# Ray0089/geometric-aware-dense-matching

Measured on AMD Instinct MI355X. Metric: rgbd_crops_per_sec_geomatch_fwd, higher is better.
Workload: dtype bf16x3/f32acc

## Files before the change

### geometric_aware_dense_matching_amd/_lib.py

```python
import ctypes
import os
import subprocess

_PKG = os.path.dirname(os.path.abspath(__file__))
LIB_PATH = os.path.join(_PKG, "libgdm_hip.so")
CSRC = os.path.join(_PKG, "csrc")

_vp = ctypes.c_void_p
_i = ctypes.c_int
_f = ctypes.c_float
_sz = ctypes.c_size_t

GDM_RANSAC_MAX_H = 4096


class KnnJob(ctypes.Structure):
    _fields_ = [("support", _vp), ("query", _vp), ("idx", _vp), ("d2", _vp),
                ("support_bstride", ctypes.c_int64), ("query_bstride", ctypes.c_int64),
                ("S", ctypes.c_int32), ("Q", ctypes.c_int32), ("K", ctypes.c_int32), ("grid_w", ctypes.c_int32)]


class PwSeg(ctypes.Structure):
    _fields_ = [("x", _vp), ("idx", _vp), ("C", ctypes.c_int32), ("n_src", ctypes.c_int32)]

# ... 22 lines not shown
    "gdm_labelstat_idx_hip": (_i, [_i, _i, _i, _i, _i, _vp, _vp, _vp, _vp]),
    "gdm_group_gather_hip": (_i, [_vp, _vp, _i, _i, _i, _i, _i, _vp, _vp]),
    "gdm_group_gather_bwd2_hip": (_i, [_vp, ctypes.c_long, _vp, _i, _i, _i, _i, _i, _vp, _vp]),
    "gdm_gather_max_hip": (_i, [_vp, _vp, _i, _i, _i, _i, _i, _vp, _vp, _vp]),
    "gdm_gather_max_bwd_hip": (_i, [_vp, _vp, _i, _i, _i, _i, _vp, _vp]),
    "gdm_rel_pos_enc_hip": (_i, [_vp, _vp, _i, _i, _i, _vp, _vp]),
    "gdm_att_pool_hip": (_i, [_vp, _vp, _i, _i, _i, _i, _vp, _vp]),
    "gdm_att_pool_bwd_hip": (_i, [_vp, _vp, _vp, _i, _i, _i, _i, _vp, _vp, _vp]),
    "gdm_match_workspace_bytes": (_sz, [_i, _i, _i]),
    "gdm_match_hip": (_i, [_vp, _vp, _i, _i, _i, _i, _i, _vp, _vp, _vp, _vp, _sz, _vp]),
    "gdm_match_rows_bytes": (_sz, [_i]),
    "gdm_match_partial_bytes": (_sz, [_i, _i]),
    "gdm_match_pack_hip": (_i, [_vp, _i, _i, _i, _i, _vp, _vp]),
    "gdm_match_pack2_hip": (_i, [_vp, _i, _i, _vp, _vp, _i, _i, _vp, _i, _i, _vp]),
    "gdm_match_packed_hip": (_i, [_vp, _vp, _i, _i, _i, _vp, _vp, _vp, _vp, _sz, _vp]),
    "gdm_seg_mask_hip": (_i, [_vp, _i, _i, _vp, _vp, _vp]),
    "gdm_spline_aggregate_hip": (_i, [_vp, _vp, _vp, _vp, _vp, _vp, _i, _i, _i, _i, _vp, _vp]),
    "gdm_spline_aggregate_bwd_hip": (_i, [_vp, _vp, _vp, _vp, _i, _i, _i, _vp, _vp]),
    "gdm_spline_direct3_hip": (_i, [_vp, _vp, _vp, _vp, _vp, _vp, _vp, _i, _i, _i, _i, _i, _vp, _vp, _vp, _vp]),
    "gdm_gemm_grouped_hip": (_i, [_vp, _vp, _vp, _vp, _i, _i, _i, _i, _vp, _vp]),
    "gdm_spline_pairs_aggregate3_hip": (_i, [_vp, _vp, _vp, _vp, _vp, _vp, _i, _i, _i, _vp, _vp, _vp, _vp]),
    "gdm_upsample_bilinear_hip": (_i, [_vp, ctypes.c_long, _i, _i, _i, _i, _vp, _vp]),
    "gdm_upsample_bilinear_bwd_hip": (_i, [_vp, ctypes.c_long, _i, _i, _i, _i, _vp, _vp]),
    "gdm_topk_rows_hip": (_i, [_vp, ctypes.c_long, _i, _i, _vp, _vp, _vp]),
    "gdm_topk_negdist_hip": (_i, [_vp, _vp, _i, _i, _i, _vp, _vp]),
    "gdm_edge_feature_hip": (_i, [_vp, _vp, _i, _i, _i, _i, _vp, _vp]),
    "gdm_edge_feature_bwd_hip": (_i, [_vp, _vp, _i, _i, _i, _i, _vp, _vp]),
    "gdm_circle_rows_fwd_hip": (_i, [_vp, _i, _i, _vp, _vp, _vp, _vp, _f, _f, _f, _vp, _vp, _vp, _vp]),
    "gdm_circle_rows_bwd_hip": (_i, [_vp, _i, _i, _vp, _vp, _vp, _vp, _f, _f, _f, _vp, _vp, _vp, _vp, _vp]),
    "gdm_circle_match_rows_bytes": (_sz, [_i]),
    "gdm_circle_match_tp_bytes": (_sz, [_i]),
    "gdm_circle_match_pack_hip": (_i, [_vp, _i, _vp, _vp, _vp, _vp]),
    "gdm_circle_match_nbr_hip": (_i, [_vp, _i, _f, _vp, _vp]),
    "gdm_circle_match_visbits_hip": (_i, [_vp, _i, _i, _vp, _vp]),
    "gdm_circle_match_nbr_items_hip": (_i, [_vp, _i, _vp, _i, _vp, _vp]),
    "gdm_circle_match_fwd2_hip": (_i, [_vp, _vp, _vp, _vp, _vp, _i, _i, _vp, _vp, _vp, _vp, _i, _vp, _i, _f, _f, _vp, _vp, _vp, _vp]),
    "gdm_circle_match_bwd2_hip": (_i, [_vp, _vp, _vp, _vp, _vp, _i, _i, _vp, _vp, _vp, _vp, _i, _vp, _i, _f, _f, _vp, _vp, _vp, _vp, _vp, _vp]),
    "gdm_circle_match_bwd_parts": (_i, [_i, _i]),
    "gdm_lfa_stage_hip": (_i, [_vp] * 13 + [_i, _i, _i, _i, _i, _f, _vp, _vp]),
    "gdm_kabsch_stats_hip": (_i, [_vp, ctypes.c_long, _i, _i, _vp, _vp, _vp, _i, _i, _i, _vp, _vp]),
    "gdm_kabsch_solve_hip": (_i, [_vp, _i, _i, _vp, _vp, _vp]),
    "gdm_ransac_workspace_bytes": (_sz, [_i, _i, _i]),
    "gdm_ransac_pose_hip": (_i, [_vp, ctypes.c_long, _i, _i, _vp, _vp, _vp, _vp, _i, _i, _i, _i, _f, ctypes.c_double, ctypes.c_uint32, _i,
                                 _vp, _sz, _vp, _vp, _vp, _vp, _vp]),
    "gdm_icp_transform_hip": (_i, [_vp, ctypes.c_long, _i, _i, _vp, _i, _i, _vp, _vp]),
    "gdm_icp_update_hip": (_i, [_vp, ctypes.c_long, _i, _i, _vp, _vp, _vp, _vp, _i, _i, _i, _f, ctypes.c_double, _i, _vp, _vp, _vp, _vp,
                                _vp]),
    "gdm_affine_act_maxk_hip": (_i, [_vp, _vp, _vp, ctypes.c_long, _i, ctypes.c_long, _i, _i, _f, _vp, _vp]),
    "gdm_prelu1_hip": (_i, [_vp, _vp, ctypes.c_long, _vp, _vp]),
    "gdm_prelu1_bwd_hip": (_i, [_vp, _vp, _vp, ctypes.c_long, _vp, _vp, _vp]),
    "gdm_affine_act_hip": (_i, [_vp, _vp, _vp, _vp, _vp, _vp, ctypes.c_long, _i, ctypes.c_long, _i, _f, _vp, _vp]),
    "gdm_upconv3x3_gather_hip": (_i, [_vp, _vp, _vp, _i, _i, _i, _i, _i, _i, _i, _f, _vp, _vp]),
    "gdm_upconv3x3_gather2_hip": (_i, [_vp, _vp, _vp, _i, _i, _i, _i, _i, _i, _i, _f, _vp, _vp, _vp]),
    "gdm_upconv3x3_gather_bwd_hip": (_i, [_vp, _i, _i, _i, _i, _i, _i, _vp, _vp]),
    "gdm_upconv_fused64_weight_bytes": (_sz, []),
    "gdm_upconv_fused64_pack_weight_hip": (_i, [_vp, _vp, _vp]),
    "gdm_upconv_fused64_hip": (_i, [_vp, _vp, _vp, _vp, _i, _i, _i, _i, _i, _i, _i, _f, _vp, _vp]),
    "gdm_psp_combine2_hip": (_i, [_vp, _vp, _i, _vp, _i, _vp, _i, _vp, _i, _vp, _i, _i, _i, _i, _vp, _vp, _vp]),
    "gdm_gather_add_affine_act2_hip": (_i, [_vp, _vp, _vp, _vp, _vp, _i, _i, _i, _i, _i, _f, _vp, _vp, _i, _vp]),
    "gdm_conv1x1_gather_add_act2_hip": (_i, [_vp, _vp, _vp, _vp, _vp, _vp, _i, _i, _i, ctypes.c_long, _i, _f, _i, _vp, _vp]),
    "gdm_conv64_gather_add_act_mfma2_hip": (_i, [_vp, _vp, _vp, _vp, _vp, _vp, _i, _i, ctypes.c_long, _i, _f, _i, _i, _vp, _vp, _i, _vp]),
    "gdm_conv3x3_act_bytes": (_sz, [_i, _i, _i, _i]),
    "gdm_conv3x3_weight_bytes": (_sz, [_i, _i]),
    "gdm_conv3x3_pack_weight_hip": (_i, [_vp, _i, _i, _vp, _vp]),
    "gdm_conv3x3_pack_act_hip": (_i, [_vp, _i, _i, _i, _i, _vp, _vp]),
    "gdm_conv3x3_packed_hip": (_i, [_vp, _vp, _vp, _vp, _vp, _i, _i, _i, _i, _i, _i, _vp, _vp]),
    "gdm_conv3x3_strided_hip": (_i, [_vp, _vp, _vp, _vp, _vp, _i, _i, _i, _i, _i, _i, _i, _vp, _vp, _vp]),
    "gdm_conv1x1_strided_hip": (_i, [_vp, _vp, _vp, _vp, _i, _i, _i, _i, _i, _i, _i, _vp, _vp]),
    "gdm_affine_relu_maxpool_hip": (_i, [_vp, _vp, _vp, _i, _i, _i, _i, _vp, _vp]),
    "gdm_conv1x1_logsoftmax_hip": (_i, [_vp, _vp, _vp, _i, _i, ctypes.c_long, _vp, _vp]),
    "gdm_pack_rows64_hip": (_i, [_vp, _i, _vp, _vp]),
    "gdm_upconv_final_points_hip": (_i, [_vp, _vp, _vp, _vp, _vp, _i, _f, _vp, _vp, _i, _i, _i, _i, _i, _i, _vp, _vp]),
    "gdm_psp_pools_hip": (_i, [_vp, ctypes.c_long, _i, _i, _vp, _vp, _vp, _vp, _vp]),
    "gdm_psp_pools_bwd_hip": (_i, [_vp, _vp, _vp, _vp, ctypes.c_long, _i, _i, _vp, _vp]),
    "gdm_conv1x1_weight_bytes": (_sz, [_i, _i]),
    "gdm_conv1x1_pack_weight_hip": (_i, [_vp, _i, _i, _vp, _vp]),
    "gdm_conv_pack_weight_dgrad_hip": (_i, [_vp, _i, _i, _i, _vp, _vp]),
    "gdm_conv1x1_packed_hip": (_i, [_vp, _vp, _vp, _vp, _i, _i, _i, _i, _i, _i, _i, _vp, _vp]),
    "gdm_depth_to_xyz_hip": (_i, [_vp, _vp, _vp, _i, _i, _i, _i, _vp, _vp]),
    "gdm_bn_sums_len": (ctypes.c_long, [_i, _i, ctypes.c_long]),
    "gdm_bn_stats_hip": (_i, [_vp, _i, _i, ctypes.c_long, _vp, _vp]),
    "gdm_bn_fwd_apply_hip": (_i, [_vp, _vp, _i, _vp, _vp, _i, _i, ctypes.c_long, _f, _f, _i, _f, _vp, _vp, _vp, _vp, _vp]),
    "gdm_bn_bwd_reduce_hip": (_i, [_vp, _vp, _vp, _i, _i, ctypes.c_long, _i, _f, _vp, _vp]),
    "gdm_bn_bwd_apply_hip": (_i, [_vp, _vp, _vp, _i, _vp, _vp, _i, _i, ctypes.c_long, _i, _f, _vp, _vp, _vp, _vp]),
    "gdm_point_heads2_hip": (_i, [_vp, _vp, _i, _vp, _vp, _i, _i, _i, _i, _vp, _vp, _vp, _vp, _i, _i, _vp, _vp, _i, _vp, _vp, _vp]),
    "gdm_pointwise2_hip": (_i, [ctypes.POINTER(PwSeg), _i, _vp, _i, _vp, _vp, _i, _i, _i, _i, _f, _vp, _i, _i, _i, _vp]),
    "gdm_pointwise_jobs_hip": (_i, [ctypes.POINTER(PwJob), _i, _i, _i, _i, _vp]),
    "gdm_pointwise_chain2_hip": (_i, [_vp, _vp, _vp, _vp, _i, _f, _vp, _vp, _vp, _i, _f, _i, _i, _i, _i, _i, _vp, _vp, _vp]),
    "gdm_stem_weight_bytes": (_sz, []),
    "gdm_stem_pack_weight_hip": (_i, [_vp, _vp, _vp]),
    "gdm_stem_hip": (_i, [_vp, _vp, _vp, _vp, _i, _i, _i, _vp, _vp, _vp]),
    "gdm_wgrad_x_bytes": (_sz, [_i, _i, _i, _i]),
    "gdm_wgrad_go_bytes": (_sz, [_i, _i, _i, _i]),
    "gdm_wgrad_pack_x_hip": (_i, [_vp, _i, _i, _i, _i, _vp, _vp]),
    "gdm_wgrad_pack_go_hip": (_i, [_vp, _i, _i, _i, _i, _vp, _vp]),
    "gdm_wgrad_x1_bytes": (_sz, [_i, _i, _i]),
    "gdm_wgrad_pack_x1_hip": (_i, [_vp, _i, _i, _i, _vp, _vp]),
    "gdm_mfma_probe_hip": (_i, [_i, _i, _i, _vp, _vp]),
    "gdm_mfma_probe_lds_hip": (_i, [_i, _i, _i, _vp, _vp]),
    "gdm_wgrad_direct_hip": (_i, [_vp, ctypes.c_long, _vp, ctypes.c_long, _i, _i, _i, _i, _i, _vp, _vp, _vp]),
    "gdm_conv1x1_packed_wb_hip": (_i, [_vp, _vp, ctypes.c_long, _i, _i, _i, _i, _i, _vp, _vp]),
    "gdm_copy_jobs_hip": (_i, [ctypes.POINTER(CopyJob), _i, _vp]),
}

_lib = None

# ... 80 lines not shown
```

### geometric_aware_dense_matching_amd/cnn.py

```python
import math
import os

import torch
import torch.nn as nn
import torch.nn.functional as F

from . import ops, settings
from .layers import act_code, cached_gemm_weight, folded_bn, fused_eval




def bn_act(bn, x, relu=None):
    if ops.bn_train_supported(x, bn):
        return ops.batch_norm_act_train(x, bn, ops.ACT_RELU if relu is not None else ops.ACT_NONE)
    y = bn(x)
    return relu(y) if relu is not None else y


def _conv3x3(cin, cout, stride=1, dilation=1):
    return nn.Conv2d(cin, cout, kernel_size=3, stride=stride, padding=dilation, dilation=dilation, bias=False)


class BasicBlock(nn.Module):
# ... 184 lines not shown
        sizes = [st[0].output_size[0] if isinstance(st[0].output_size, (tuple, list)) else st[0].output_size for st in self.stages]
        if (settings.USE_SPLIT_PSP_TRAIN and feats.is_cuda and feats.dtype == torch.float32 and sizes == [1, 2, 3, 6] and ops.psp_pools_supported(h, w)
                and (h * w) % 4 == 0 and feats.shape[0] * self.bottleneck.out_channels <= 65535 and h <= 64 and w <= 64):
            B, F_ = feats.shape[0], feats.shape[1]
            w2 = self.bottleneck.weight.view(self.bottleneck.out_channels, -1)
            g = ops.wx(w2[:, 4 * F_:], feats.reshape(B, F_, h * w)).view(B, -1, h, w)
            pools = ops.psp_pools(feats)
            ys = []
            for k, st in enumerate(self.stages):
                m = w2[:, k * F_:(k + 1) * F_] @ st[1].weight.view(F_, F_)
                ys.append(ops.wx(m, pools[k].reshape(B, F_, sizes[k] * sizes[k])).view(B, -1, sizes[k], sizes[k]))
            return ops.psp_combine_train(g, ys, self.bottleneck.bias)
        priors = [ops.upsample_bilinear(stage(feats), (h, w)) for stage in self.stages] + [feats]
        return self.relu(self.bottleneck(torch.cat(priors, 1)))


class Upsample2x(nn.Module):

    def forward(self, x):
        return ops.upsample_bilinear(x, (x.shape[2] * 2, x.shape[3] * 2))


class PSPUpsample(nn.Module):
    def __init__(self, cin, cout):
        super().__init__()
        self.conv = nn.Sequential(Upsample2x(), nn.Conv2d(cin, cout, 3, padding=1), nn.BatchNorm2d(cout), nn.PReLU())

    def _tap_major_weight(self):
        w = self.conv[1].weight
        key = (w._version, w.data_ptr())
        cache = self.__dict__.get("_gdm_wt")
        if cache is None or cache[0] != key:
            with torch.no_grad():
                wt = w.permute(2, 3, 0, 1).reshape(9 * w.shape[0], w.shape[1]).contiguous()
            cache = (key, wt)
            self.__dict__["_gdm_wt"] = cache
        return cache[1]

    def forward(self, x):
        if fused_eval(x, self):
            code = act_code(self.conv[3])
            conv = self.conv[1]
            if code is not None and x.shape[0] * conv.out_channels <= 65535 and conv.in_channels >= settings.UPCONV_MIN_CIN:
                Bx, Cin, Hx, Wx = x.shape
                if settings.USE_FUSED_UPCONV and Cin == 64 and conv.out_channels == 64 and Hx >= 2 and Wx >= 2 and Bx <= 65535:
                    w = conv.weight
                    key = (w._version, w.data_ptr())
                    cache = self.__dict__.get("_gdm_fused64")
                    if cache is None or cache[0] != key:
                        cache = (key, ops.upconv_fused64_pack_weight(w))
                        self.__dict__["_gdm_fused64"] = cache
                    scale, shift = folded_bn(self.conv[2], conv.bias)
                    return ops.upconv_fused64(x, cache[1], scale, shift, (Hx * 2, Wx * 2), code[0], code[1])
                if settings.USE_MFMA_GEMM and ops.gemm_supported(Cin, 9 * conv.out_channels, Hx * Wx):
                    wpk, c9 = cached_gemm_weight(self, "tap", self._tap_major_weight, (conv.weight,))
                    z = ops.gemm_bf16x3_map(x, wpk, c9)
                else:
                    z = ops.wx(self._tap_major_weight(), x.reshape(Bx, Cin, Hx * Wx)).view(Bx, -1, Hx, Wx)
                scale, shift = folded_bn(self.conv[2], conv.bias)
                return ops.upconv3x3_gather(z, scale, shift, conv.out_channels, (x.shape[2] * 2, x.shape[3] * 2), code[0], code[1],
                                            packed=settings.USE_MFMA_GEMM and settings.USE_PACKED_PRODUCERS and conv.out_channels % 128 == 0)
        act = self.conv[3]
        if x.is_cuda and isinstance(act, nn.PReLU) and act.weight.numel() == 1 and x.dtype == torch.float32:
            conv = self.conv[1]
            if settings.USE_LOWRES_UPCONV_TRAIN and ops.upconv_train_supported(x.shape[0], conv.out_channels) and conv.in_channels >= settings.UPCONV_MIN_CIN:
                Bx, Cin, Hx, Wx = x.shape
                w9 = conv.weight.permute(2, 3, 0, 1).reshape(9 * conv.out_channels, Cin)
                z = ops.wx(w9, x.reshape(Bx, Cin, Hx * Wx)).view(Bx, -1, Hx, Wx)
                y = bn_act(self.conv[2], ops.upconv3x3_gather_train(z, conv.bias, conv.out_channels, (Hx * 2, Wx * 2)))
            else:
                y = bn_act(self.conv[2], conv(self.conv[0](x)))
            if y.numel() % 4 == 0:
                return ops.prelu1(y, act.weight)
            return act(y)
        return self.conv(x)


class FinalStage(nn.Sequential):

    def forward(self, x):
        conv = self[0]
        if fused_eval(x, self) and conv.in_channels == 64 and conv.out_channels == 64 and x.shape[0] <= 65535:
            return ops.conv1x1_logsoftmax(x, conv.weight, conv.bias)
        if self.training and ops.conv1x1_train_supported(conv, x):
            return self[1](ops.conv1x1_train(conv, x))
        return nn.Sequential.forward(self, x)


class PSPNet(nn.Module):

    def __init__(self):
        super().__init__()
        self.feats = ResNet18Trunk()
        self.psp = PSPModule(512, 1024, (1, 2, 3, 6))
        self.drop_1 = nn.Dropout2d(p=0.3)
        self.up_1 = PSPUpsample(1024, 256)
        self.up_2 = PSPUpsample(256, 64)
        self.up_3 = PSPUpsample(64, 64)
        self.drop_2 = nn.Dropout2d(p=0.15)
        self.final = FinalStage(nn.Conv2d(64, 64, kernel_size=1), nn.LogSoftmax(dim=1))
```

### geometric_aware_dense_matching_amd/ops.py

```python
import ctypes
import os

import torch

from . import _lib, settings
from ._lib import KnnJob, check

MATCH_BF16X3 = 0
MATCH_F32 = 1


def _stream():
    return torch.cuda.current_stream().cuda_stream


_side_streams = {}


def side_stream(device, which=0):
    key = (device.index if device.index is not None else torch.cuda.current_device(), which)
    st = _side_streams.get(key)
    if st is None:
        st = torch.cuda.Stream(device=device)
        _side_streams[key] = st
# ... 687 lines not shown
    if not bn.affine or bn.momentum is None or not bn.track_running_stats:
        return False
    B, C = x.shape[0], x.shape[1]
    inner = x.numel() // max(B * C, 1)
    return B * C <= 65535 and inner >= 4 and inner % 4 == 0 and x.data_ptr() % 16 == 0 and B * inner > 1


def batch_norm_act_train(x, bn, act=ACT_NONE, slope=0.0):
    y = _BatchNormAct.apply(x, bn.weight, bn.bias, bn.running_mean, bn.running_var, bn.eps, bn.momentum, act, slope, _sync_group(bn))
    if bn.num_batches_tracked is not None:
        if _bn_counters is not None:
            _bn_counters.append(bn.num_batches_tracked)
        else:
            bn.num_batches_tracked.add_(1)
    return y


_bn_counters = None


class batched_bn_counters:

    def __enter__(self):
        global _bn_counters
        self.prev, _bn_counters = _bn_counters, []
        return self

    def __exit__(self, *exc):
        global _bn_counters
        pending, _bn_counters = _bn_counters, self.prev
        if pending:
            torch._foreach_add_(pending, 1)
        return False


def upconv3x3_gather(z, scale, shift, cout, out_size, act=ACT_NONE, slope=0.0, packed=False):
    z = _dev(z, torch.float32, "z")
    B, c9, H, W = z.shape
    assert c9 == 9 * cout
    OH, OW = int(out_size[0]), int(out_size[1])
    out = torch.empty((B, cout, OH, OW), dtype=torch.float32, device=z.device)
    if (packed and (cout == 64 or cout % 128 == 0) and OW % 32 == 0 and (B * OH * OW) % 256 == 0 and B * cout // 8 <= 65535
            and (OH, OW) == (2 * H, 2 * W)):
        opk = PackedAct(_packed_buffer(B, cout, OH, OW, z.device), (B, cout, OH, OW))
        check(_lib.lib().gdm_upconv3x3_gather2_hip(z.data_ptr(), scale.data_ptr(), shift.data_ptr(), B, cout, H, W, OH, OW, act,
                                                   float(slope), out.data_ptr(), opk.buf.data_ptr(), _stream()), "gdm_upconv3x3_gather2_hip")
        out._gdm_packed = opk
        return out
    check(_lib.lib().gdm_upconv3x3_gather_hip(z.data_ptr(), scale.data_ptr(), shift.data_ptr(), B, cout, H, W, OH, OW, act,
                                              float(slope), out.data_ptr(), _stream()), "gdm_upconv3x3_gather_hip")
    return out


def upconv_fused64_pack_weight(weight):
    w = _dev(weight.detach(), torch.float32, "weight")
    if tuple(w.shape) != (64, 64, 3, 3):
        raise ValueError("upconv_fused64_pack_weight: weight must be [64,64,3,3], got %s" % (tuple(w.shape),))
    L = _lib.lib()
    wpk = torch.empty(L.gdm_upconv_fused64_weight_bytes(), dtype=torch.uint8, device=w.device)
    check(L.gdm_upconv_fused64_pack_weight_hip(w.data_ptr(), wpk.data_ptr(), _stream()), "gdm_upconv_fused64_pack_weight_hip")
    return wpk


def upconv_fused64(x, wpk, scale, shift, out_size, act=0, slope=0.0):
    x = _dev(x, torch.float32, "x")
    B, C, H, W = x.shape
    OH, OW = int(out_size[0]), int(out_size[1])
    out = torch.empty((B, C, OH, OW), dtype=torch.float32, device=x.device)
    check(_lib.lib().gdm_upconv_fused64_hip(x.data_ptr(), wpk.data_ptr(), scale.data_ptr(), shift.data_ptr(), B, C, H, W, OH, OW, act,
                                            float(slope), out.data_ptr(), _stream()), "gdm_upconv_fused64_hip")
    return out


class _UpconvGather(torch.autograd.Function):

    @staticmethod
    def forward(ctx, z, bias, cout, OH, OW):
        z = z.contiguous()
        B, c9, H, W = z.shape
        ones = torch.ones(cout, dtype=torch.float32, device=z.device)
        shift = bias.detach().contiguous() if bias is not None else torch.zeros(cout, dtype=torch.float32, device=z.device)
        out = torch.empty((B, cout, OH, OW), dtype=torch.float32, device=z.device)
        check(_lib.lib().gdm_upconv3x3_gather_hip(z.data_ptr(), ones.data_ptr(), shift.data_ptr(), B, cout, H, W, OH, OW, ACT_NONE, 0.0,
                                                  out.data_ptr(), _stream()), "gdm_upconv3x3_gather_hip")
        ctx.shape = (B, cout, H, W, OH, OW)
        ctx.has_bias = bias is not None
        return out

    @staticmethod
    def backward(ctx, go):
        B, cout, H, W, OH, OW = ctx.shape
        go = go.contiguous()
        gz = torch.empty((B, 9 * cout, H, W), dtype=torch.float32, device=go.device)
        check(_lib.lib().gdm_upconv3x3_gather_bwd_hip(go.data_ptr(), B, cout, H, W, OH, OW, gz.data_ptr(), _stream()),
              "gdm_upconv3x3_gather_bwd_hip")
        return gz, (channel_sum(go) if ctx.has_bias else None), None, None, None


def upconv3x3_gather_train(z, bias, cout, out_size):
    z = _dev(z, torch.float32, "z")
    assert z.shape[1] == 9 * cout
    return _UpconvGather.apply(z, bias, cout, int(out_size[0]), int(out_size[1]))


def wx(w2d, x3):
    if torch.is_grad_enabled() and (w2d.requires_grad or x3.requires_grad) and x3.is_cuda and x3.dtype == torch.float32:
# ... 843 lines not shown
```

### geometric_aware_dense_matching_amd/settings.py

```python
import os


def _flag(name, default="1"):
    return os.environ.get(name, default) != "0"


USE_MFMA_CONV = _flag("GDM_MFMA_CONV")
USE_MFMA_CONV_TRAIN = _flag("GDM_MFMA_CONV_TRAIN")
USE_MFMA_GEMM = _flag("GDM_MFMA_GEMM")
USE_FUSED_UPCONV = _flag("GDM_FUSED_UPCONV")
USE_LOWRES_UPCONV_TRAIN = _flag("GDM_LOWRES_UPCONV_TRAIN")
USE_SPLIT_PSP_TRAIN = _flag("GDM_SPLIT_PSP_TRAIN")
USE_FUSED_LFA = _flag("GDM_FUSED_LFA")
USE_GROUPED_SPLINE = _flag("GDM_GROUPED_SPLINE")
USE_FUSED_BN_TRAIN = _flag("GDM_FUSED_BN_TRAIN")
USE_FUSED_SYNCBN = _flag("GDM_FUSED_SYNCBN")
USE_FUSED_MATCH_LOSS = _flag("GDM_FUSED_MATCH_LOSS")
USE_SIDE_STREAMS = _flag("GDM_SIDE_STREAMS", "0")
USE_SPARSE_FINAL = _flag("GDM_SPARSE_FINAL")
USE_FUSED_HEADS = _flag("GDM_FUSED_HEADS")
USE_MFMA_STRIDED = _flag("GDM_MFMA_STRIDED")
USE_POINTWISE = _flag("GDM_POINTWISE")
USE_OWN_STEM = _flag("GDM_OWN_STEM")
USE_GEMM_CONV1X1_TRAIN = _flag("GDM_GEMM_CONV1X1_TRAIN")
USE_MFMA_WGRAD = _flag("GDM_MFMA_WGRAD")
USE_MFMA_GEMM_TRAIN = _flag("GDM_MFMA_GEMM_TRAIN")
USE_GATHERED_FINAL = _flag("GDM_GATHERED_FINAL")
USE_DIRECT_WGRAD = _flag("GDM_DIRECT_WGRAD")
USE_FUSED_ADAM = _flag("GDM_FUSED_ADAM")
USE_POINTWISE_TRAIN = _flag("GDM_POINTWISE_TRAIN")
USE_POINT_CHAIN = _flag("GDM_POINT_CHAIN")
USE_PSP_JOBS = _flag("GDM_PSP_JOBS")
USE_PACKED_PRODUCERS = _flag("GDM_PACKED_PRODUCERS")
USE_TWO_STREAM_PIPELINE = _flag("GDM_TWO_STREAM_PIPELINE")
MESH_FORK_LATE = os.environ.get("GDM_MESH_FORK_LATE", "1") != "0"
PACK_MESH_ROWS = os.environ.get("GDM_PACK_MESH_ROWS", "1") != "0"
SIDE_PARTS = os.environ.get("GDM_SIDE_PARTS", "mesh,point,pyr").split(",")
STATIC_MATCH_ROWS = _flag("GDM_STATIC_MATCH_ROWS", "0")
UPCONV_MIN_CIN = int(os.environ.get("GDM_UPCONV_MIN_CIN", "0"))
SYNCBN_MIN_WORLD = 2

ALL_SWITCHES = ("USE_MFMA_CONV", "USE_MFMA_CONV_TRAIN", "USE_MFMA_GEMM", "USE_FUSED_UPCONV", "USE_LOWRES_UPCONV_TRAIN",
                "USE_SPLIT_PSP_TRAIN", "USE_FUSED_LFA", "USE_GROUPED_SPLINE", "USE_FUSED_BN_TRAIN", "USE_FUSED_SYNCBN",
                "USE_FUSED_MATCH_LOSS", "USE_SIDE_STREAMS", "USE_SPARSE_FINAL", "USE_FUSED_HEADS", "USE_MFMA_STRIDED", "USE_POINTWISE", "USE_OWN_STEM", "USE_GEMM_CONV1X1_TRAIN", "USE_MFMA_WGRAD", "USE_MFMA_GEMM_TRAIN", "USE_GATHERED_FINAL", "USE_DIRECT_WGRAD", "USE_PSP_JOBS", "USE_POINT_CHAIN", "USE_POINTWISE_TRAIN")
SPLIT_BF16_SWITCHES = ("USE_MFMA_CONV", "USE_MFMA_GEMM", "USE_FUSED_UPCONV", "USE_SPARSE_FINAL", "USE_FUSED_HEADS", "USE_MFMA_STRIDED",
                       "USE_OWN_STEM")
```

### include/gdm.h

```cpp
#ifndef GDM_H
#define GDM_H

#include <stddef.h>
#include <stdint.h>

#ifdef __cplusplus
extern "C" {
#endif

#define GDM_EINVAL (-1)
#define GDM_ENOMEM (-2)

const char* gdm_last_error(void);
int gdm_version(void);


void gdm_knn_batch(const float* batch_data, size_t batch_size, size_t npts, size_t dim,
                   const float* queries, size_t nqueries, size_t K, long* batch_indices);

int gdm_knn_batch_hip(const float* support, const float* query, int B, int S, int Q, int K,
                      int32_t* idx, float* d2, void* stream);

typedef struct gdm_knn_job {
    const float* support;
// ... 91 lines not shown
                            const float* lse_p, const float* lse_n, const float* grad_rows, float* dsim, void* stream);

size_t gdm_circle_match_rows_bytes(int n);
size_t gdm_circle_match_tp_bytes(int n);
int gdm_circle_match_pack_hip(const float* x, int n, void* rows, void* tp, float* rowsum, void* stream);
int gdm_circle_match_nbr_hip(const float* xyz, int M, float radius, uint32_t* nbr, void* stream);
int gdm_circle_match_visbits_hip(const uint8_t* vis, int B, int M, uint32_t* bits, void* stream);
int gdm_circle_match_nbr_items_hip(const float* xyz, int M, const float* rad , int B, uint32_t* nbr, void* stream);
int gdm_circle_match_fwd2_hip(const void* xrows, const void* xtp, const float* xpad, const void* yrows, const void* ytp,
                              int R, int M, const int32_t* g, const int32_t* c2, const int32_t* item,
                              const uint32_t* nbr, int nbr_per_item, const uint32_t* visb, int pad_e0, float gamma, float m,
                              float* lse_p, float* lse_n, float* loss, void* stream);
int gdm_circle_match_bwd2_hip(const void* xrows, const void* xtp, const float* xpad, const void* yrows, const void* ytp,
                              int R, int M, const int32_t* g, const int32_t* c2, const int32_t* item,
                              const uint32_t* nbr, int nbr_per_item, const uint32_t* visb, int pad_e0, float gamma, float m,
                              const float* lse_p, const float* lse_n, const float* coef, float* gx, float* gy_part, void* stream);
int gdm_circle_match_bwd_parts(int R, int M);

int gdm_lfa_stage_hip(const float* xyz, const int32_t* idx, const float* feat, const float* w1t, const float* s1, const float* b1,
                      const float* w2t, const float* s2, const float* b2, const float* wft, const float* wmt, const float* sm,
                      const float* bm, int B, int n, int K, int D, int OUT, float slope, float* out, void* stream);

int gdm_kabsch_stats_hip(const float* scene_xyz, long scene_bstride, int pt_stride, int ch_stride, const float* model_xyz,
                         const int32_t* best_idx, const uint8_t* mask, int B, int N, int M, double* out, void* stream);

int gdm_kabsch_solve_hip(const double* stats, int B, int min_points, float* RT, uint8_t* valid, void* stream);

#define GDM_RANSAC_MAX_H 4096
size_t gdm_ransac_workspace_bytes(int B, int N, int H);
int gdm_ransac_pose_hip(const float* scene_xyz, long scene_bstride, int pt_stride, int ch_stride, const float* model_xyz,
                        const int32_t* best_idx, const uint8_t* mask, const double* stats, int B, int N, int M, int H,
                        float match_err, double fix_percent, uint32_t seed, int min_points, void* workspace, size_t workspace_bytes,
                        float* RT, uint8_t* valid, int32_t* counts, int32_t* winner, void* stream);

int gdm_icp_transform_hip(const float* scene_xyz, long scene_bstride, int pt_stride, int ch_stride, const float* RT, int B, int N,
                          float* query, void* stream);
int gdm_icp_update_hip(const float* scene_xyz, long scene_bstride, int pt_stride, int ch_stride, const float* model_xyz,
                       const int32_t* nn, const float* d2, const uint8_t* mask, int B, int N, int M, float reject_dist,
                       double tolerance, int min_points, float* RT, uint8_t* active, int32_t* iters, double* err, void* stream);

int gdm_affine_act_maxk_hip(const float* x, const float* scale, const float* shift, long planes, int C, long n, int K, int act,
                            float slope, float* out, void* stream);

int gdm_prelu1_hip(const float* x, const float* slope, long n, float* y, void* stream);
int gdm_prelu1_bwd_hip(const float* x, const float* grad_out, const float* slope, long n, float* grad_x, float* grad_slope, void* stream);

int gdm_affine_act_hip(const float* x, const float* scale, const float* shift, const float* res, const float* res_scale,
                       const float* res_shift, long planes, int C, long inner, int act, float slope, float* y, void* stream);

int gdm_upconv3x3_gather_hip(const float* z, const float* scale, const float* shift, int B, int Cout, int H, int W,
                             int OH, int OW, int act, float slope, float* out, void* stream);
int gdm_upconv3x3_gather2_hip(const float* z, const float* scale, const float* shift, int B, int Cout, int H, int W,
                              int OH, int OW, int act, float slope, float* out, void* outpk, void* stream);
int gdm_upconv3x3_gather_bwd_hip(const float* grad_out, int B, int Cout, int H, int W, int OH, int OW, float* grad_z, void* stream);
size_t gdm_upconv_fused64_weight_bytes(void);
int gdm_upconv_fused64_pack_weight_hip(const float* w, void* wpk, void* stream);
int gdm_upconv_fused64_hip(const float* x, const void* wpk, const float* scale, const float* shift, int B, int C, int H, int W,
                           int OH, int OW, int act, float slope, float* out, void* stream);

int gdm_psp_combine2_hip(const float* g, const float* y1, int s1, const float* y2, int s2, const float* y3, int s3,
                         const float* y4, int s4, const float* bias, int B, int C, int H, int W, float* out, void* outpk, void* stream);
int gdm_gather_add_affine_act2_hip(const float* x, const float* t, const int32_t* idx, const float* scale, const float* shift,
                                   int B, int C, int n, int m, int act, float slope, float* y, void* y_packed, int W, void* stream);
int gdm_conv1x1_gather_add_act2_hip(const float* x, const float* wt, const float* t, const int32_t* idx, const float* scale,
                                    const float* shift, int B, int C, int n, long m, int act, float slope, int pixel_major,
                                    float* y, void* stream);
int gdm_conv64_gather_add_act_mfma2_hip(const float* x, const void* wpk, const float* t, const int32_t* idx, const float* scale,
                                        const float* shift, int B, int n, long m, int act, float slope, int pixel_major,
                                        int t_point_major, float* y, void* ypk, int W, void* stream);

size_t gdm_conv3x3_act_bytes(int B, int Cin, int H, int W);
size_t gdm_conv3x3_weight_bytes(int Cout, int Cin);
int gdm_conv3x3_pack_weight_hip(const float* w, int Cout, int Cin, void* wpk, void* stream);
int gdm_conv3x3_pack_act_hip(const float* x, int B, int Cin, int H, int W, void* xpk, void* stream);
int gdm_conv3x3_packed_hip(const void* xpk, const void* wpk, const float* scale, const float* shift, const float* res,
                           int B, int Cin, int Cout, int H, int W, int act, float* out, void* stream);
int gdm_conv3x3_strided_hip(const void* xpk, const void* wpk, const float* scale, const float* shift, const float* res,
                            int B, int Cin, int Cout, int H, int W, int stride, int act, float* out, void* outpk, void* stream);
int gdm_conv1x1_strided_hip(const void* xpk, const void* wpk, const float* scale, const float* shift,
                            int B, int Cin, int Cout, int H, int W, int stride, int act, float* out, void* stream);

int gdm_affine_relu_maxpool_hip(const float* x, const float* scale, const float* shift, int B, int C, int H, int W, float* y, void* stream);
int gdm_conv1x1_logsoftmax_hip(const float* x, const float* w, const float* bias, int B, int C, long hw, float* out, void* stream);
int gdm_pack_rows64_hip(const float* w, int R, void* out, void* stream);
int gdm_upconv_final_points_hip(const float* xpm, const int32_t* choose, const void* wpk, const float* scale, const float* shift,
                                int act, float slope, const void* wfpk, const float* fbias, int B, int H, int W, int OH, int OW,
                                int N, float* out, void* stream);
int gdm_psp_pools_hip(const float* x, long planes, int H, int W, float* o1, float* o2, float* o3, float* o6, void* stream);
int gdm_psp_pools_bwd_hip(const float* g1, const float* g2, const float* g3, const float* g6, long planes, int H, int W,
                          float* grad_x, void* stream);

size_t gdm_conv1x1_weight_bytes(int Cout, int Cin);
int gdm_conv1x1_pack_weight_hip(const float* w, int Cout, int Cin, void* wpk, void* stream);
int gdm_conv_pack_weight_dgrad_hip(const float* w, int Cout, int Cin, int taps, void* wpk, void* stream);
int gdm_conv1x1_packed_hip(const void* xpk, const void* wpk, const float* scale, const float* shift,
                           int B, int Cin, int Cout, int H, int W, int act, int pixel_major, float* out, void* stream);

int gdm_depth_to_xyz_hip(const float* depth, const float* K, const int32_t* origin, int B, int H, int W, int S,
                         float* out, void* stream);

long gdm_bn_sums_len(int B, int C, long inner);
int gdm_bn_stats_hip(const float* x, int B, int C, long inner, double* sums, void* stream);
int gdm_bn_fwd_apply_hip(const float* x, const double* sums, int groups, const float* weight, const float* bias, int B, int C, long inner, float eps,
                         float momentum, int act, float slope, float* saved, float* running_mean, float* running_var, float* y, void* stream);
int gdm_bn_bwd_reduce_hip(const float* x, const float* grad_out, const float* saved, int B, int C, long inner, int act, float slope,
                          double* sums, void* stream);
// ... 58 lines not shown
```

Measured before the change: 5075.

## Fuse tap-major upconv GEMM with bilinear upsample gather in one MFMA kernel

Adds a HIP kernel that computes the per-tap 3x3 conv products on the low-resolution input with bf16x3 MFMA and keeps them on chip. It then performs the bilinear-upsample tap gather, the folded BN affine and the activation from shared memory, optionally writing packed output. This avoids materialising the 9*Cout-channel intermediate tensor in global memory and the separate gather launch. It only applies to W=32 and Cin a multiple of 128, and is gated by a new settings flag. It adds band-overlap recomputation of rows and a large shared-memory footprint, which limits occupancy.

```diff
diff --git a/geometric_aware_dense_matching_amd/_lib.py b/geometric_aware_dense_matching_amd/_lib.py
--- a/geometric_aware_dense_matching_amd/_lib.py
+++ b/geometric_aware_dense_matching_amd/_lib.py
@@ -98,6 +98,7 @@
     "gdm_affine_act_hip": (_i, [_vp, _vp, _vp, _vp, _vp, _vp, ctypes.c_long, _i, ctypes.c_long, _i, _f, _vp, _vp]),
     "gdm_upconv3x3_gather_hip": (_i, [_vp, _vp, _vp, _i, _i, _i, _i, _i, _i, _i, _f, _vp, _vp]),
     "gdm_upconv3x3_gather2_hip": (_i, [_vp, _vp, _vp, _i, _i, _i, _i, _i, _i, _i, _f, _vp, _vp, _vp]),
+    "gdm_upconv3x3_tap_fused_hip": (_i, [_vp, _vp, _vp, _vp, _i, _i, _i, _i, _i, _i, _f, _vp, _vp, _vp]),
     "gdm_upconv3x3_gather_bwd_hip": (_i, [_vp, _i, _i, _i, _i, _i, _i, _vp, _vp]),
     "gdm_upconv_fused64_weight_bytes": (_sz, []),
     "gdm_upconv_fused64_pack_weight_hip": (_i, [_vp, _vp, _vp]),
diff --git a/geometric_aware_dense_matching_amd/cnn.py b/geometric_aware_dense_matching_amd/cnn.py
--- a/geometric_aware_dense_matching_amd/cnn.py
+++ b/geometric_aware_dense_matching_amd/cnn.py
@@ -260,6 +260,12 @@
                         self.__dict__["_gdm_fused64"] = cache
                     scale, shift = folded_bn(self.conv[2], conv.bias)
                     return ops.upconv_fused64(x, cache[1], scale, shift, (Hx * 2, Wx * 2), code[0], code[1])
+                packed = settings.USE_MFMA_GEMM and settings.USE_PACKED_PRODUCERS and conv.out_channels % 128 == 0
+                if (settings.USE_MFMA_GEMM and settings.USE_TAP_FUSED_UPCONV
+                        and ops.upconv_tap_fused_supported(Bx, Cin, conv.out_channels, Hx, Wx, (2 * Hx, 2 * Wx))):
+                    wpk, _ = cached_gemm_weight(self, "tapblk", lambda: ops.upconv_tap_block_weight(conv.weight), (conv.weight,))
+                    scale, shift = folded_bn(self.conv[2], conv.bias)
+                    return ops.upconv3x3_tap_fused(x, wpk, scale, shift, conv.out_channels, code[0], code[1], packed=packed)
                 if settings.USE_MFMA_GEMM and ops.gemm_supported(Cin, 9 * conv.out_channels, Hx * Wx):
                     wpk, c9 = cached_gemm_weight(self, "tap", self._tap_major_weight, (conv.weight,))
                     z = ops.gemm_bf16x3_map(x, wpk, c9)
@@ -267,7 +273,7 @@
                     z = ops.wx(self._tap_major_weight(), x.reshape(Bx, Cin, Hx * Wx)).view(Bx, -1, Hx, Wx)
                 scale, shift = folded_bn(self.conv[2], conv.bias)
                 return ops.upconv3x3_gather(z, scale, shift, conv.out_channels, (x.shape[2] * 2, x.shape[3] * 2), code[0], code[1],
-                                            packed=settings.USE_MFMA_GEMM and settings.USE_PACKED_PRODUCERS and conv.out_channels % 128 == 0)
+                                            packed=packed)
         act = self.conv[3]
         if x.is_cuda and isinstance(act, nn.PReLU) and act.weight.numel() == 1 and x.dtype == torch.float32:
             conv = self.conv[1]
diff --git a/geometric_aware_dense_matching_amd/csrc/gdm_upconv_tap.hip b/geometric_aware_dense_matching_amd/csrc/gdm_upconv_tap.hip
--- /dev/null
+++ b/geometric_aware_dense_matching_amd/csrc/gdm_upconv_tap.hip
@@ -0,0 +1,289 @@
+#include "gdm_common.h"
+
+namespace {
+
+typedef __attribute__((ext_vector_type(8))) __bf16 bf16x8;
+typedef __attribute__((ext_vector_type(4))) unsigned u32x4;
+typedef __attribute__((ext_vector_type(4))) float f32x4;
+
+constexpr int ROWB = 512;
+constexpr int UT_W = 32;
+constexpr int UT_T = 8;
+constexpr int UT_THREADS = UT_T * 64;
+constexpr int UT_NPH = 2;
+constexpr int UT_NCB = 9;
+constexpr int UT_NS = 4;
+constexpr int UT_PANEL = UT_NCB * 16 * ROWB;
+constexpr int UT_CS = 20;
+constexpr int UT_STAGE = 3 * UT_T * UT_W * UT_CS * 4;
+constexpr int UT_SMEM = 2 * UT_PANEL > UT_STAGE ? 2 * UT_PANEL : UT_STAGE;
+
+__device__ __forceinline__ int swz(int col, int ch) { return col * ROWB + (((ch & 16) | ((ch ^ col) & 15)) << 4); }
+
+}
+
+__host__ __device__ static inline void upconv_tap_band(int k, int H, int& r0, int& r1)
+{
+    r0 = k == 0 ? 0 : (UT_T - 1) + (k - 1) * (UT_T - 2);
+    r1 = (H - r0 <= UT_T - 1) ? H : r0 + (k == 0 ? UT_T - 1 : UT_T - 2);
+}
+
+static int upconv_tap_bands(int H)
+{
+    int k = 0, r0, r1;
+    do upconv_tap_band(k++, H, r0, r1); while (r1 < H);
+    return k;
+}
+
+namespace {
+
+template <int ACT>
+__global__ __launch_bounds__(UT_THREADS) void upconv_tap_fused_kernel(const unsigned char* __restrict__ xpk, const unsigned char* __restrict__ wpk,
+                                                                      const float* __restrict__ scale, const float* __restrict__ shift,
+                                                                      int Cin, int Cout, int H, int nband, float rh, float rw, float slope,
+                                                                      float* __restrict__ out, unsigned char* __restrict__ ypk)
+{
+    extern __shared__ __attribute__((aligned(16))) unsigned char smem[];
+    constexpr int W = UT_W, NS = UT_NS, NPH = UT_NPH, NCB = UT_NCB, PANEL = UT_PANEL;
+    constexpr int UG = 3, NPR = NCB / UG;
+    const int tid = threadIdx.x, lane = tid & 63;
+    const int wave = __builtin_amdgcn_readfirstlane(tid >> 6);
+    const int l16 = lane & 15, kg = lane >> 4;
+    const int nchunk = Cin / 128;
+    const int b = blockIdx.x / nband, band = blockIdx.x - b * nband;
+    const int cb0 = blockIdx.y * 16;
+    int r0, r1;
+    upconv_tap_band(band, H, r0, r1);
+    const int c0 = max(r0 - 1, 0);
+    const long plane = (long)(H + 2) * (W + 2);
+
+    const __amdgpu_buffer_rsrc_t xr = __builtin_amdgcn_make_buffer_rsrc(const_cast<unsigned char*>(xpk), (short)0, 0x7ffffff0, 0x00020000);
+    int avoff[NPH];
+    const int yrow = min(c0 + wave, H - 1);
+#pragma unroll
+    for (int ph = 0; ph < NPH; ++ph) avoff[ph] = (int)(((long)kg * plane + (long)(yrow + 1) * (W + 2) + 16 * ph + l16 + 1) * 16);
+    u32x4 ahi[NS][NPH], alo[NS][NPH];
+    const int a_base = (int)((long)b * nchunk * 32 * plane * 16);
+    const int a_chunk = (int)(32 * plane * 16);
+    const int sstride = (int)(4 * plane * 16), lostride = (int)(16 * plane * 16);
+    auto load_a = [&](int r, int S) {
+#pragma unroll
+        for (int ph = 0; ph < NPH; ++ph) {
+            ahi[S][ph] = __builtin_bit_cast(u32x4, __builtin_amdgcn_raw_buffer_load_b128(xr, avoff[ph], r + S * sstride, 0));
+            alo[S][ph] = __builtin_bit_cast(u32x4, __builtin_amdgcn_raw_buffer_load_b128(xr, avoff[ph], r + S * sstride + lostride, 0));
+        }
+    };
+    const __amdgpu_buffer_rsrc_t wr = __builtin_amdgcn_make_buffer_rsrc(const_cast<unsigned char*>(wpk), (short)0, 0x7ffffff0, 0x00020000);
+    const int w_base = blockIdx.y * (NCB * 16) * ROWB;
+    const int w_panel = ((9 * Cout + 127) & ~127) * ROWB;
+    constexpr int NPIECE = PANEL / 1024 / 8;
+    const int hrow = lane >> 5, sl = lane & 31;
+    const int col15 = (2 * wave + hrow) & 15;
+    const int glds_voff = wave * 1024 + hrow * 512 + (((sl & 16) | ((sl ^ col15) & 15)) << 4);
+    typedef __attribute__((address_space(3))) void* lds_void_ptr;
+    auto stage_glds = [&](int src, int buf) {
+#pragma unroll
+        for (int i = 0; i < NPIECE; ++i)
+            __builtin_amdgcn_raw_ptr_buffer_load_lds(wr, (lds_void_ptr)(smem + buf * PANEL + (i * 8 + wave) * 1024), 16, glds_voff, src + i * 8192, 0, 0);
+    };
+
+    f32x4 acc[NPH][NCB];
+#pragma unroll
+    for (int ph = 0; ph < NPH; ++ph)
+#pragma unroll
+        for (int cb = 0; cb < NCB; ++cb)
+#pragma unroll
+            for (int i = 0; i < 4; ++i) acc[ph][cb][i] = 0.f;
+
+    constexpr int LATE = 1;
+    stage_glds(w_base, 0);
+    int rcur = a_base;
+#pragma unroll
+    for (int S = 0; S < NS - LATE; ++S) load_a(rcur, S);
+    int rnext = nchunk > 1 ? a_base + a_chunk : a_base, wnext = nchunk > 1 ? w_base + w_panel : w_base;
+    for (int it = 0; it < nchunk; ++it) {
+        __syncthreads();
+        const bool more = it + 1 < nchunk;
+        const unsigned char* base = smem + (it & 1) * PANEL;
+        constexpr int PF = 2;
+        constexpr int NU = NPR * NS;
+        u32x4 fh[PF + 1][UG], fl[PF + 1][UG];
+        auto frag_load = [&](int un) {
+            const int S = un / NPR, pr = un % NPR, slot = un % (PF + 1);
+#pragma unroll
+            for (int j = 0; j < UG; ++j) {
+                const int col = (UG * pr + j) * 16 + l16;
+                fh[slot][j] = *reinterpret_cast<const u32x4*>(base + swz(col, 4 * S + kg));
+                fl[slot][j] = *reinterpret_cast<const u32x4*>(base + swz(col, 16 + 4 * S + kg));
+            }
+        };
+#pragma unroll
+        for (int un = 0; un < PF; ++un) frag_load(un);
+#pragma unroll
+        for (int u = 0; u < NU; ++u) {
+            const int S = u / NPR, pr = u % NPR, slot = u % (PF + 1);
+            if (u + PF < NU) frag_load(u + PF);
+#pragma unroll
+            for (int ph = 0; ph < NPH; ++ph) {
+                const bf16x8 ah = __builtin_bit_cast(bf16x8, ahi[S][ph]);
+                const bf16x8 al = __builtin_bit_cast(bf16x8, alo[S][ph]);
+#pragma unroll
+                for (int j = 0; j < UG; ++j) {
+                    f32x4 c = acc[ph][UG * pr + j];
+                    c = __builtin_amdgcn_mfma_f32_16x16x32_bf16(ah, __builtin_bit_cast(bf16x8, fl[slot][j]), c, 0, 0, 0);
+                    c = __builtin_amdgcn_mfma_f32_16x16x32_bf16(al, __builtin_bit_cast(bf16x8, fh[slot][j]), c, 0, 0, 0);
+                    c = __builtin_amdgcn_mfma_f32_16x16x32_bf16(ah, __builtin_bit_cast(bf16x8, fh[slot][j]), c, 0, 0, 0);
+                    acc[ph][UG * pr + j] = c;
+                }
+            }
+            if (pr == NPR - 1 && S < NS - LATE) load_a(rnext, S);
+            if (u == 0) {
+                if (more) stage_glds(wnext, (it + 1) & 1);
+#pragma unroll
+                for (int S2 = NS - LATE; S2 < NS; ++S2) load_a(rcur, S2);
+            }
+#pragma unroll
+            for (int i = 0; i < 3 * UG * NPH; ++i) {
+                __builtin_amdgcn_sched_group_barrier(0x008, 1, 0);
+                if (u + PF < NU && (i % NPH) == 0 && i < 2 * UG * NPH) __builtin_amdgcn_sched_group_barrier(0x100, 1, 0);
+            }
+            __builtin_amdgcn_sched_barrier(0);
+        }
+        rcur = rnext;
+        const int nx = it + 2 < nchunk ? it + 2 : it + 1 < nchunk ? it + 1 : it;
+        rnext = a_base + nx * a_chunk;
+        wnext = w_base + nx * w_panel;
+    }
+
+    const int OH = 2 * H, OW = 2 * W;
+    const int X = lane;
+    const int nrow = 2 * (r1 - r0);
+    int cx0[3], cx1[3];
+    float clx[3], chx[3];
+    bool cok[3];
+#pragma unroll
+    for (int d = 0; d < 3; ++d) {
+        const int xx = X + d - 1;
+        cok[d] = xx >= 0 && xx < OW;
+        const float sx = rw * (float)max(xx, 0);
+        const int x0 = min((int)sx, W - 1);
+        cx0[d] = x0;
+        cx1[d] = min(x0 + 1, W - 1);
+        clx[d] = sx - (float)x0;
+        chx[d] = 1.f - clx[d];
+    }
+    float o[2][16];
+#pragma unroll
+    for (int s = 0; s < 2; ++s)
+#pragma unroll
+        for (int c = 0; c < 16; ++c) o[s][c] = 0.f;
+    float* zs = reinterpret_cast<float*>(smem);
+#pragma unroll
+    for (int ky = 0; ky < 3; ++ky) {
+        __syncthreads();
+#pragma unroll
+        for (int kx = 0; kx < 3; ++kx)
+#pragma unroll
+            for (int ph = 0; ph < NPH; ++ph)
+#pragma unroll
+                for (int r = 0; r < 4; ++r)
+                    zs[((kx * UT_T + wave) * W + 16 * ph + 4 * kg + r) * UT_CS + l16] = acc[ph][3 * ky + kx][r] + 0.f;
+        __syncthreads();
+        const int dy = ky - 1;
+#pragma unroll
+        for (int s = 0; s < 2; ++s) {
+            const int yl = wave + 8 * s;
+            const int yy = 2 * r0 + yl + dy;
+            if (yl >= nrow || yy < 0 || yy >= OH) continue;
+            const float sy = rh * (float)yy;
+            const int y0 = min((int)sy, H - 1);
+            const float ly = sy - (float)y0, hy = 1.f - ly;
+            const int ya = min(max(y0 - c0, 0), UT_T - 1), yb = min(max(min(y0 + 1, H - 1) - c0, 0), UT_T - 1);
+#pragma unroll
+            for (int kx = 0; kx < 3; ++kx) {
+                if (!cok[kx]) continue;
+                const float lx = clx[kx], hx = chx[kx];
+                const float* p00 = zs + ((kx * UT_T + ya) * W + cx0[kx]) * UT_CS;
+                const float* p01 = zs + ((kx * UT_T + ya) * W + cx1[kx]) * UT_CS;
+                const float* p10 = zs + ((kx * UT_T + yb) * W + cx0[kx]) * UT_CS;
+                const float* p11 = zs + ((kx * UT_T + yb) * W + cx1[kx]) * UT_CS;
+#pragma unroll
+                for (int q = 0; q < 4; ++q) {
+                    const float4 a00 = *reinterpret_cast<const float4*>(p00 + 4 * q), a01 = *reinterpret_cast<const float4*>(p01 + 4 * q);
+                    const float4 a10 = *reinterpret_cast<const float4*>(p10 + 4 * q), a11 = *reinterpret_cast<const float4*>(p11 + 4 * q);
+                    const float v00[4] = {a00.x, a00.y, a00.z, a00.w}, v01[4] = {a01.x, a01.y, a01.z, a01.w};
+                    const float v10[4] = {a10.x, a10.y, a10.z, a10.w}, v11[4] = {a11.x, a11.y, a11.z, a11.w};
+#pragma unroll
+                    for (int j = 0; j < 4; ++j) {
+                        const float top = fmaf(lx, v01[j], hx * v00[j]);
+                        const float bot = fmaf(lx, v11[j], hx * v10[j]);
+                        o[s][4 * q + j] = fmaf(ly, bot, fmaf(hy, top, o[s][4 * q + j]));
+                    }
+                }
+            }
+        }
+    }
+    const int Cpk = (Cout + 127) / 128;
+    const long pplane = (long)(OH + 2) * (OW + 2);
+#pragma unroll
+    for (int s = 0; s < 2; ++s) {
+        const int yl = wave + 8 * s;
+        if (yl >= nrow) continue;
+        const int Y = 2 * r0 + yl;
+        float v[16];
+#pragma unroll
+        for (int c = 0; c < 16; ++c) {
+            float t = o[s][c] * scale[cb0 + c] + shift[cb0 + c];
+            if (ACT == 1) t = fmaxf(t, 0.f);
+            if (ACT == 2) t = t > 0.f ? t : t * slope;
+            v[c] = t;
+            out[(((long)b * Cout + cb0 + c) * OH + Y) * OW + X] = t;
+        }
+        if (ypk) {
+#pragma unroll
+            for (int g = 0; g < 2; ++g) {
+                const int cg = cb0 + 8 * g, chunk = cg / 128, q = (cg % 128) / 8;
+                unsigned char* op = ypk + ((((long)b * Cpk + chunk) * 32 + q) * pplane + (long)(Y + 1) * (OW + 2) + X + 1) * 16;
+                unsigned hi[4], lo[4];
+#pragma unroll
+                for (int i = 0; i < 4; ++i) gdm_split2(v[8 * g + 2 * i], v[8 * g + 2 * i + 1], hi[i], lo[i]);
+                *reinterpret_cast<uint4*>(op) = make_uint4(hi[0], hi[1], hi[2], hi[3]);
+                *reinterpret_cast<uint4*>(op + 16 * pplane * 16) = make_uint4(lo[0], lo[1], lo[2], lo[3]);
+            }
+        }
+    }
+}
+
+}
+
+extern "C" int gdm_upconv3x3_tap_fused_hip(const void* xpk, const void* wpk, const float* scale, const float* shift, int B, int Cin, int Cout,
+                                           int H, int W, int act, float slope, float* out, void* outpk, void* stream)
+{
+    GDM_CHECK_ARG(xpk && wpk && scale && shift && out, "gdm_upconv3x3_tap_fused_hip: NULL pointer");
+    GDM_CHECK_ARG(B >= 1 && Cin >= 128 && Cin % 128 == 0 && Cout >= 16 && Cout % 16 == 0 && (long)B * Cout <= 65535 && W == UT_W && H >= 2,
+                  "gdm_upconv3x3_tap_fused_hip: bad shape B=%d Cin=%d Cout=%d %dx%d (Cin a multiple of 128, Cout of 16, W = %d, H >= 2)",
+                  B, Cin, Cout, H, W, UT_W);
+    GDM_CHECK_ARG(act >= 0 && act <= 2, "gdm_upconv3x3_tap_fused_hip: act=%d", act);
+    GDM_CHECK_ARG(((uintptr_t)outpk & 15) == 0 && (!outpk || Cout == 64 || Cout % 128 == 0),
+                  "gdm_upconv3x3_tap_fused_hip: packed output unaligned or Cout=%d not 64 / a multiple of 128", Cout);
+    const long act_bytes = (long)B * (H + 2) * (W + 2) * (Cin / 128) * ROWB;
+    const long w_bytes = (long)(Cin / 128) * ((9L * Cout + 127) & ~127L) * ROWB;
+    GDM_CHECK_ARG(act_bytes < (1L << 31) && w_bytes < (1L << 31),
+                  "gdm_upconv3x3_tap_fused_hip: packed operand (%ld B) or weights (%ld B) not below 2 GiB", act_bytes, w_bytes);
+    const int nband = upconv_tap_bands(H);
+    GDM_CHECK_ARG((long)B * nband <= 0x7fffffffL, "gdm_upconv3x3_tap_fused_hip: too many bands");
+    static bool attr = false;
+    if (!attr) {
+        (void)hipFuncSetAttribute((const void*)upconv_tap_fused_kernel<0>, hipFuncAttributeMaxDynamicSharedMemorySize, UT_SMEM);
+        (void)hipFuncSetAttribute((const void*)upconv_tap_fused_kernel<1>, hipFuncAttributeMaxDynamicSharedMemorySize, UT_SMEM);
+        (void)hipFuncSetAttribute((const void*)upconv_tap_fused_kernel<2>, hipFuncAttributeMaxDynamicSharedMemorySize, UT_SMEM);
+        attr = true;
+    }
+    const float rh = (float)(H - 1) / (float)(2 * H - 1), rw = (float)(W - 1) / (float)(2 * W - 1);
+    const dim3 grid(B * nband, Cout / 16);
+    hipStream_t s = (hipStream_t)stream;
+#define UTF(A) hipLaunchKernelGGL(upconv_tap_fused_kernel<A>, grid, dim3(UT_THREADS), UT_SMEM, s, (const unsigned char*)xpk, (const unsigned char*)wpk, scale, shift, Cin, Cout, H, nband, rh, rw, slope, out, (unsigned char*)outpk)
+    if (act == 0) UTF(0); else if (act == 1) UTF(1); else UTF(2);
+#undef UTF
+    return gdm_launch_status("upconv_tap_fused_kernel");
+}
diff --git a/geometric_aware_dense_matching_amd/ops.py b/geometric_aware_dense_matching_amd/ops.py
--- a/geometric_aware_dense_matching_amd/ops.py
+++ b/geometric_aware_dense_matching_amd/ops.py
@@ -763,6 +763,34 @@
     return out
 
 
+def upconv_tap_fused_supported(B, cin, cout, H, W, out_size):
+    act_bytes = B * (H + 2) * (W + 2) * (cin // 128) * 512 if cin > 0 else 0
+    w_bytes = (cin // 128) * ((9 * cout + 127) // 128 * 128) * 512 if cin > 0 else 0
+    return (W == 32 and H >= 2 and tuple(out_size) == (2 * H, 2 * W) and B >= 1 and cin >= 128 and cin % 128 == 0
+            and cout >= 16 and cout % 16 == 0 and B * cout <= 65535 and act_bytes < 2 ** 31 and w_bytes < 2 ** 31)
+
+
+def upconv_tap_block_weight(weight):
+    co, ci = weight.shape[0], weight.shape[1]
+    return weight.reshape(co // 16, 16, ci, 9).permute(0, 3, 1, 2).reshape(9 * co, ci).contiguous()
+
+
+def upconv3x3_tap_fused(x, wpk, scale, shift, cout, act=ACT_NONE, slope=0.0, packed=False):
+    B, Cin, H, W = x.shape
+    xp = getattr(x, "_gdm_packed", None)
+    if not (isinstance(xp, PackedAct) and xp.shape == (B, Cin, H, W)):
+        xp = conv3x3_pack_act(x)
+    OH, OW = 2 * H, 2 * W
+    out = torch.empty((B, cout, OH, OW), dtype=torch.float32, device=xp.buf.device)
+    opk = PackedAct(_packed_buffer(B, cout, OH, OW, out.device), (B, cout, OH, OW)) if packed else None
+    check(_lib.lib().gdm_upconv3x3_tap_fused_hip(xp.buf.data_ptr(), wpk.data_ptr(), scale.data_ptr(), shift.data_ptr(), B, Cin, cout, H, W,
+                                                 act, float(slope), out.data_ptr(), opk.buf.data_ptr() if packed else None, _stream()),
+          "gdm_upconv3x3_tap_fused_hip")
+    if packed:
+        out._gdm_packed = opk
+    return out
+
+
 def upconv_fused64_pack_weight(weight):
     w = _dev(weight.detach(), torch.float32, "weight")
     if tuple(w.shape) != (64, 64, 3, 3):
diff --git a/geometric_aware_dense_matching_amd/settings.py b/geometric_aware_dense_matching_amd/settings.py
--- a/geometric_aware_dense_matching_amd/settings.py
+++ b/geometric_aware_dense_matching_amd/settings.py
@@ -9,6 +9,7 @@
 USE_MFMA_CONV_TRAIN = _flag("GDM_MFMA_CONV_TRAIN")
 USE_MFMA_GEMM = _flag("GDM_MFMA_GEMM")
 USE_FUSED_UPCONV = _flag("GDM_FUSED_UPCONV")
+USE_TAP_FUSED_UPCONV = _flag("GDM_TAP_FUSED_UPCONV")
 USE_LOWRES_UPCONV_TRAIN = _flag("GDM_LOWRES_UPCONV_TRAIN")
 USE_SPLIT_PSP_TRAIN = _flag("GDM_SPLIT_PSP_TRAIN")
 USE_FUSED_LFA = _flag("GDM_FUSED_LFA")
diff --git a/include/gdm.h b/include/gdm.h
--- a/include/gdm.h
+++ b/include/gdm.h
@@ -167,6 +167,8 @@
                              int OH, int OW, int act, float slope, float* out, void* stream);
 int gdm_upconv3x3_gather2_hip(const float* z, const float* scale, const float* shift, int B, int Cout, int H, int W,
                               int OH, int OW, int act, float slope, float* out, void* outpk, void* stream);
+int gdm_upconv3x3_tap_fused_hip(const void* xpk, const void* wpk, const float* scale, const float* shift, int B, int Cin, int Cout,
+                                int H, int W, int act, float slope, float* out, void* outpk, void* stream);
 int gdm_upconv3x3_gather_bwd_hip(const float* grad_out, int B, int Cout, int H, int W, int OH, int OW, float* grad_z, void* stream);
 size_t gdm_upconv_fused64_weight_bytes(void);
 int gdm_upconv_fused64_pack_weight_hip(const float* w, void* wpk, void* stream);
```

Result: faster. 5132, median of 6 (+1.1%).
